# yakir12/PawsomeTracker.jl

Measured on AMD Instinct MI355X. Metric: DoG+argmax frames/s, 1080p 256x256 windows batch 4096; % HBM roofline @1/8 GPU, higher is better.
Workload: dtype f32

## Files before the change

pawsometracker.jl_amd/csrc/dog_prune.hpp:

```cpp
#pragma once
#include "dog_roll.hpp"
#include "dog_prune_words.hpp"
#include "dog_prune_publish.hpp"

namespace pdog {

struct PruneGeo {
    LaunchGeo g;
    double kinv;
    float tmax;
    int darker;
    unsigned long long *stat;
    uint64_t *host;
    PruneJob *jobs;
    const uint32_t *wq;
};

constexpr int PRUNE_NT = 256;
constexpr int PRUNE_B = 8;
constexpr int PRUNE_PHASES = 9;
constexpr int PRUNE_REFINE_MAX_SPAN = 32;
__host__ __device__ inline int prune_refine_pitch(int NS) { return (NS + 3) / 4 * 4; }
struct PruneLds { size_t cell, E, segd, strd, S, R, patch, root, hull2, total; };
__host__ __device__ inline PruneLds prune_lds(int n1, int n2, int L, int nslots, bool refine = false)
// ... 60 lines not shown

    const int ncols = g.nthin ? g.thin_x0 : g.n2;
    const int ws = min(TW, ncols);
    auto slot_cols = [&](int sl, int &c0, int &c1) {
        const bool strip = sl < g.nstrips;
        c0 = strip ? ((ncols >= TW) ? min(sl * TW, ncols - TW) : 0) : g.thin_x0 + (sl - g.nstrips);
        c1 = c0 + (strip ? ws + L - 1 : L);
    };
    auto seg_id = [&](int c) {
        int id = 0;
        for (int sl = 0; sl < g.nslots; ++sl) {
            int c0, c1;
            slot_cols(sl, c0, c1);
            id += (c0 <= c) + (c1 <= c);
        }
        return id;
    };
    auto row_in = [&](int gi) { return gi >= 0 && gi < g.fh; };
    const bool narrow8 = NARROW && g.fw < 8, narrow4 = NARROW && g.fw < 4;
    const unsigned rs = (unsigned)g.row_stride;
    auto frame_at = [&](int gi, int gjc) { return frame + ((unsigned long long)(unsigned)pw_clamp_row(gi, g.fh) * rs + (unsigned)gjc); };
    auto tile_word = [&](int gi, int gj, uint32_t in) -> uint32_t {
        uint32_t w = 0;
        if (in == 0xffffffffu) {
            __builtin_memcpy(&w, frame + (long long)gi * g.row_stride + gj, 4);
        } else if (in) {
#pragma unroll
            for (int i = 0; i < 4; ++i)
                if ((in >> (8 * i)) & 1u) w |= (uint32_t)frame[(long long)gi * g.row_stride + gj + i] << (8 * i);
        }
        return w;
    };

    const int nitems = nsub * ncx;
    auto cell_load = [&](int band, int cx, uint32_t (&w)[2 * CH]) {
        const int gj = wj0 + 8 * cx, gi0 = ti0 + band * CH;
        if (!narrow8) {
            const uint8_t *src = frame_at(gi0, pw_clamp_col(gj, g.fw, 8));
#pragma unroll
            for (int r = 0; r < CH; ++r) {
                __builtin_memcpy(&w[2 * r], src, 8);
                src += (unsigned)(gi0 + r) < (unsigned)(g.fh - 1) ? rs : 0u;
            }
        } else {
            const uint32_t in_a = pw_mask(gj, 0, g.fw), in_b = pw_mask(gj + 4, 0, g.fw);
            for (int r = 0; r < CH; ++r) {
                const bool rin = row_in(gi0 + r);
                w[2 * r] = tile_word(gi0 + r, gj, rin ? in_a : 0u);
                w[2 * r + 1] = tile_word(gi0 + r, gj + 4, rin ? in_b : 0u);
            }
        }
    };

    if (tid == 0) s_nstr = 0;
    int dc;
    uint32_t cur[2 * CH];
    {
        constexpr int DCN = 1024 / NT;
        const int tH = NA, tW = TWin;
        int sv[DCN];
        bool sin[DCN];
#pragma unroll
        for (int j = 0; j < DCN; ++j) {
            const int k = tid + j * NT;
            const int gi = ti0 + (int)(((long long)(k >> 5) * tH) >> 5), gj = wj0 + (int)(((long long)(k & 31) * tW) >> 5);
            sin[j] = row_in(gi) && gj >= 0 && gj < g.fw;
            sv[j] = *frame_at(gi, min(max(gj, 0), g.fw - 1));
        }
        {
            const int it0 = min(tid, nitems - 1), band0 = it0 / ncx;
            cell_load(band0, it0 - band0 * ncx, cur);
        }
        for (int i = tid; i < nsub * nseg * 2; i += NT) S[i] = 0;
        if (refine) {
            for (int i = tid; i <= nsub; i += NT) root[i * rp + ncx] = 0;
            for (int i = tid; i < ncx; i += NT) root[nsub * rp + i] = 0;
        }
        int sum = 0;
#pragma unroll
        for (int j = 0; j < DCN; ++j) sum += sin[j] ? sv[j] : g.fill;
        sum = wave_sum(sum);
        if (lane == 0) s_sum[wave] = sum;
        __syncthreads();
        int tot = 0;
        for (int w = 0; w < NW; ++w) tot += s_sum[w];
        dc = __builtin_amdgcn_readfirstlane(dc_from_sum(tot, g.fill));
    }
    for (int d = tid; d < TQ2; d += NT) {
        int sd = -1;
        if (4 * d < TWin) {
            const int first = seg_id(4 * d), last = seg_id(min(4 * d + 3, TWin - 1));
            if (first == last) sd = first;
            else strd[atomicAdd(&s_nstr, 1)] = (unsigned short)d;
        }
        segd[d] = (short)sd;
    }
    __syncthreads();
    PRUNE_STAMP(0);

    PwAcc ext = pw_init();
    auto cell_sums = [&](int band, int cx, const uint32_t (&w)[2 * CH]) {
        const int col0 = 8 * cx, gj = wj0 + col0, a0 = band * CH, gi0 = ti0 + a0, nr = min(CH, NA - a0);
        const uint32_t cnt_a = pw_mask(col0, 0, TWin), cnt_b = pw_mask(col0 + 4, 0, TWin);
        uint32_t s2a = 0, s1a = 0, s2b = 0, s1b = 0;
        if (nr == CH && gi0 >= 0 && gi0 + CH <= g.fh && gj >= 0 && gj + 8 <= g.fw) {
#pragma unroll
            for (int r = 0; r < CH; ++r) {
                const PwWords xa = pw_words(w[2 * r], 0xffffffffu, cnt_a, fill4), xb = pw_words(w[2 * r + 1], 0xffffffffu, cnt_b, fill4);
                pw_moments(s2a, s1a, xa.wz);
                pw_extremes(ext, xa);
                pw_moments(s2b, s1b, xb.wz);
                pw_extremes(ext, xb);
            }
        } else {
            const uint32_t in_a = pw_mask(gj, 0, g.fw), in_b = pw_mask(gj + 4, 0, g.fw);
            if ((in_a | in_b) == 0u || gi0 >= g.fh || gi0 + nr <= 0) {
                const PwWords xa = pw_words(0u, 0u, cnt_a, fill4), xb = pw_words(0u, 0u, cnt_b, fill4);
                pw_moments(s2a, s1a, xa.wz);
                pw_moments(s2b, s1b, xb.wz);
                s2a *= (uint32_t)nr; s1a *= (uint32_t)nr; s2b *= (uint32_t)nr; s1b *= (uint32_t)nr;
                pw_extremes(ext, xa);
                pw_extremes(ext, xb);
            } else {
                const PwShift sh = narrow8 ? PwShift{0u, 0u} : pw_shift(pw_clamp_col(gj, g.fw, 8) - gj, 8);
#pragma unroll
                for (int r = 0; r < CH; ++r) {
                    const bool rin = row_in(gi0 + r), rc = r < nr;
                    const uint64_t v = pw_rebuild64((uint64_t)w[2 * r] | ((uint64_t)w[2 * r + 1] << 32), sh);
                    const PwWords xa = pw_words((uint32_t)v, rin ? in_a : 0u, rc ? cnt_a : 0u, fill4);
                    const PwWords xb = pw_words((uint32_t)(v >> 32), rin ? in_b : 0u, rc ? cnt_b : 0u, fill4);
                    pw_moments(s2a, s1a, xa.wz);
                    pw_extremes(ext, xa);
                    pw_moments(s2b, s1b, xb.wz);
                    pw_extremes(ext, xb);
                }
            }
        }
        const int npx = nr * min(TWin - col0, 8);
        cell[band * ncx + cx] = pw_sum(s1a + s1b, npx, dc);
        if (refine) root[band * rp + cx] = (unsigned short)pw_root16(pw_energy(s2a + s2b, s1a + s1b, npx, dc));
        const int sda = segd[2 * cx], sdb = segd[2 * cx + 1];
        unsigned *Sb = S + 2 * band * nseg;
        if (sda == sdb) {
            if (sda >= 0) { atomicAdd(Sb + 2 * sda, s2a + s2b); atomicAdd(Sb + 2 * sda + 1, s1a + s1b); }
        } else {
            if (sda >= 0) { atomicAdd(Sb + 2 * sda, s2a); atomicAdd(Sb + 2 * sda + 1, s1a); }
            if (sdb >= 0) { atomicAdd(Sb + 2 * sdb, s2b); atomicAdd(Sb + 2 * sdb + 1, s1b); }
        }
    };
    if (tid < nitems) {
        int band = tid / ncx, cx = tid - band * ncx;
        const int bstep = NT / ncx, cstep = NT - bstep * ncx;
        for (int it = tid + NT; it < nitems; it += NT) {
            int nband = band + bstep, ncell = cx + cstep;
            if (ncell >= ncx) { ncell -= ncx; ++nband; }
            uint32_t nxt[2 * CH];
            cell_load(nband, ncell, nxt);
            cell_sums(band, cx, cur);
#pragma unroll
            for (int i = 0; i < 2 * CH; ++i) cur[i] = nxt[i];
            band = nband;
            cx = ncell;
        }
        cell_sums(band, cx, cur);
    }
    {
        const int pmax = wave_reduce_bits(pw_pmax(ext), [](int a, int c) { return a > c ? a : c; });
        const int pmin = wave_min(pw_pmin(ext));
        if (lane == 0) { s_pmax[wave] = pmax; s_pmin[wave] = pmin; }
    }
    __syncthreads();
    PRUNE_STAMP(1);

    for (int j = 0, nstr = s_nstr; j < nstr; ++j) {
        const int d = strd[j], gj = wj0 + 4 * d;
        const uint32_t in_cols = pw_mask(gj, 0, g.fw);
        const int gjc = narrow4 ? 0 : pw_clamp_col(gj, g.fw, 4);
        const PwShift sh = narrow4 ? PwShift{0u, 0u} : pw_shift(gjc - gj, 4);
        for (int t = tid; t < 4 * nsub; t += NT) {
            const int band = t >> 2, col = 4 * d + (t & 3), a0 = band * CH, nr = min(CH, NA - a0);
            if (col >= TWin) continue;
            const uint32_t counted = pw_mask(4 * d, col, col + 1);
            uint32_t w[CH];
            if (!narrow4) {
#pragma unroll
                for (int r = 0; r < CH; ++r) __builtin_memcpy(&w[r], frame_at(ti0 + a0 + r, gjc), 4);
            } else {
                for (int r = 0; r < CH; ++r) w[r] = tile_word(ti0 + a0 + r, gj, row_in(ti0 + a0 + r) ? in_cols & counted : 0u);
// ... 291 lines not shown
```

pawsometracker.jl_amd/csrc/dog_prune_words.hpp:

```cpp
#pragma once
#include <stdint.h>

#if defined(__HIPCC__) || defined(__CUDACC__)
#define PW_HD __host__ __device__ inline
#else
#define PW_HD inline
#endif

namespace pdog {

PW_HD uint32_t pw_low_bytes(int n) { return n >= 4 ? 0xffffffffu : n <= 0 ? 0u : (1u << (8 * n)) - 1u; }
PW_HD uint32_t pw_mask(int col0, int lo, int hi) { return pw_low_bytes(hi - col0) & ~pw_low_bytes(lo - col0); }

struct PwWords { uint32_t wz, wo; };
PW_HD PwWords pw_words(uint32_t w, uint32_t in_frame, uint32_t counted, uint32_t fill4)
{
    const uint32_t keep = in_frame & counted;
    const uint32_t z = (w & keep) | (fill4 & counted & ~keep);
    return PwWords{z, z | ~counted};
}

PW_HD int pw_clamp_col(int gj, int fw, int width) { return gj < 0 ? 0 : gj > fw - width ? fw - width : gj; }
PW_HD int pw_clamp_row(int gi, int fh) { return gi < 0 ? 0 : gi > fh - 1 ? fh - 1 : gi; }
struct PwShift { unsigned up, down; };
// ... 8 lines not shown
#if defined(__HIP_DEVICE_COMPILE__)
typedef unsigned short pw_us2 __attribute__((ext_vector_type(2)));
PW_HD uint32_t pw_dot4(uint32_t a, uint32_t b, uint32_t c) { return __builtin_amdgcn_udot4(a, b, c, false); }
PW_HD uint32_t pw_pk_max(uint32_t a, uint32_t b)
{
    return __builtin_bit_cast(uint32_t, __builtin_elementwise_max(__builtin_bit_cast(pw_us2, a), __builtin_bit_cast(pw_us2, b)));
}
PW_HD uint32_t pw_pk_min(uint32_t a, uint32_t b)
{
    return __builtin_bit_cast(uint32_t, __builtin_elementwise_min(__builtin_bit_cast(pw_us2, a), __builtin_bit_cast(pw_us2, b)));
}
PW_HD uint32_t pw_mul24(uint32_t a, uint32_t b) { return __umul24(a, b); }
PW_HD float pw_sqrt_est(float x) { return __builtin_amdgcn_sqrtf(x); }
#else
PW_HD uint32_t pw_mul24(uint32_t a, uint32_t b) { return a * b; }
PW_HD float pw_sqrt_est(float x) { return __builtin_sqrtf(x); }
PW_HD uint32_t pw_dot4(uint32_t a, uint32_t b, uint32_t c)
{
    for (int i = 0; i < 4; ++i) c += ((a >> (8 * i)) & 0xffu) * ((b >> (8 * i)) & 0xffu);
    return c;
}
PW_HD uint32_t pw_pk_max(uint32_t a, uint32_t b)
{
    const uint32_t al = a & 0xffffu, bl = b & 0xffffu, ah = a >> 16, bh = b >> 16;
    return (al > bl ? al : bl) | ((ah > bh ? ah : bh) << 16);
}
PW_HD uint32_t pw_pk_min(uint32_t a, uint32_t b)
{
    const uint32_t al = a & 0xffffu, bl = b & 0xffffu, ah = a >> 16, bh = b >> 16;
    return (al < bl ? al : bl) | ((ah < bh ? ah : bh) << 16);
}
#endif

constexpr uint32_t PW_EVEN = 0x00ff00ffu, PW_ODD = 0xff00ff00u;

struct PwAcc {
    uint32_t s2, s1;
    uint32_t max_e, max_o, min_e, min_o;
};
PW_HD PwAcc pw_init() { return PwAcc{0u, 0u, 0u, 0u, PW_EVEN, PW_ODD}; }

PW_HD void pw_moments(uint32_t &s2, uint32_t &s1, uint32_t wz)
{
    s2 = pw_dot4(wz, wz, s2);
    s1 = pw_dot4(wz, 0x01010101u, s1);
}
PW_HD void pw_extremes(PwAcc &a, PwWords x)
{
    a.max_e = pw_pk_max(a.max_e, x.wz & PW_EVEN);
    a.max_o = pw_pk_max(a.max_o, x.wz & PW_ODD);
    a.min_e = pw_pk_min(a.min_e, x.wo & PW_EVEN);
    a.min_o = pw_pk_min(a.min_o, x.wo & PW_ODD);
}
PW_HD void pw_update(PwAcc &a, PwWords x)
{
    pw_moments(a.s2, a.s1, x.wz);
    pw_extremes(a, x);
}

PW_HD int pw_pmax(const PwAcc &a)
{
    const uint32_t e = (a.max_e & 0xffffu) > (a.max_e >> 16) ? (a.max_e & 0xffffu) : (a.max_e >> 16);
    const uint32_t o = (a.max_o & 0xffffu) > (a.max_o >> 16) ? (a.max_o & 0xffffu) : (a.max_o >> 16);
    return (int)(e > (o >> 8) ? e : (o >> 8));
}
PW_HD int pw_pmin(const PwAcc &a)
{
    const uint32_t e = (a.min_e & 0xffffu) < (a.min_e >> 16) ? (a.min_e & 0xffffu) : (a.min_e >> 16);
    const uint32_t o = (a.min_o & 0xffffu) < (a.min_o >> 16) ? (a.min_o & 0xffffu) : (a.min_o >> 16);
    return (int)(e < (o >> 8) ? e : (o >> 8));
}

PW_HD uint32_t pw_energy(uint32_t s2, uint32_t s1, int n, int dc) { return (s2 + (uint32_t)n * (uint32_t)(dc * dc)) - 2u * (uint32_t)dc * s1; }
PW_HD uint32_t pw_root16(uint32_t e)
{
    const uint32_t e256 = e << 8;
    uint32_t r = (uint32_t)(16.0f * pw_sqrt_est((float)e));
    r += pw_mul24(r, r) < e256;
    r += pw_mul24(r, r) < e256;
    return r;
}
PW_HD int pw_sum(uint32_t s1, int n, int dc) { return (int)s1 - n * dc; }
PW_HD int pw_V(int pmax, int pmin, int dc)
{
    const int up = pmax - dc, dn = dc - pmin, v = up > dn ? up : dn;
    return v > 0 ? v : 0;
}

}
```

pawsometracker.jl_amd/csrc/pawsome_dog.hip:

```cpp
#include "pdog_host.hpp"
#include "pdog_mailbox.hpp"
#include "pdog_policy.hpp"
#include "pdog_plan.hpp"
#include "dog_kernels.hpp"
#include "dog_roll.hpp"
#include "dog_prune.hpp"
#include "dog_twopass.hpp"
#include "dog_fused.hpp"
#include "dog_exact.hpp"
#include "dog_tiled.hpp"
#include "dog_measure.hpp"
#include "dog_step.hpp"

#include <algorithm>
#include <cmath>
#include <cstdio>
#include <cstring>
#include <cstdlib>
#include <atomic>
#include <chrono>
#include <map>
#include <memory>
#include <mutex>
#include <thread>
// ... 200 lines not shown
    hipEvent_t ev_h2d[kSlots] = {nullptr, nullptr, nullptr}, ev_used[kSlots] = {nullptr, nullptr, nullptr};
};

}

struct pdog_tracker {
    int device = 0;
    Switches sw;
    hipEvent_t ev_switch = nullptr;
    int fh = 0, fw = 0, r1 = 0, r2 = 0, n1 = 0, n2 = 0, L = 0, fill = 0, darker = 0;
    double tw = 0, sigma = 0;
    Plan plan;
    const VariantKernels *kern = nullptr;
    int fused_resident = 0, tiled_resident = 0;
    DeviceBuffer<int32_t> d_chain_tmp;
    pdog::StagedTable table;
    TiledRun tiled_run;
    DeviceBuffer<f2> d_V;
    MapPolicy map_policy;
    unsigned win_launched = 0;
    PrunePolicy prune_policy;
    double K_norm = 0;
    DeviceBuffer<unsigned long long> d_prune_stat;
    DeviceBuffer<uint32_t> d_refine_wq;
    int last_prune_n = 0, last_prune_nstrips = 0;
    DeviceBuffer<PruneJob> d_prune_jobs;
    int last_n = 0, last_nslots = 0;
    DeviceBuffer<float> d_map;
    DeviceBuffer<int> d_dc;
    DeviceBuffer<int> d_counter;
    hipStream_t own_stream = nullptr, stream = nullptr;
    hipStream_t aux_stream = nullptr;
    hipEvent_t ev_fork = nullptr, ev_join = nullptr;
    DeviceBuffer<f2> d_taps_row, d_taps_col;
    DeviceBuffer<f2> d_taps_roll;
    DeviceBuffer<f2> d_fold_r;
    DeviceBuffer<float> d_part_val, d_part_sec;
    DeviceBuffer<unsigned long long> d_part_mask;
    DeviceBuffer<int> d_part_idx;
    bool exact = true;
    bool exact_all = false;
    std::vector<double> h_gp, h_gm;
    double F_sym_int = 0, F_sym_sep = 0, F_ring = 0, F_rescan = 0;
    DeviceBuffer<double> d_K64;
    DeviceBuffer<double> d_g64;
    DeviceBuffer<RefineParams> d_rp;
    double exact_T64 = 0.0;
    DeviceBuffer<unsigned long long> d_ref_stat;
    DeviceBuffer<uint8_t> d_frame;
    DeviceBuffer<int32_t> d_small;
    PinnedBuffer<Mailbox> h_pinned{hipHostMallocMapped | hipHostMallocCoherent};
    int32_t ticket = 0;
    DeviceBuffer<float> d_resp;
    PinnedBuffer<uint8_t> h_tile{hipHostMallocMapped};
    Ingest ingest;
    pdog::PeaksState peaks;
    pdog::GroupWalkState exclusive;
    pdog::GroupWalkState motion;
    bool motion_lds = false;
    pdog::PredictState predict;

    ~pdog_tracker()
    {
        (void)hipSetDevice(device);
        if (stream) (void)hipStreamSynchronize(stream);
        for (hipStream_t s : {ingest.stream, aux_stream})
            if (s) { (void)hipStreamSynchronize(s); (void)hipStreamDestroy(s); }
        for (int k = 0; k < Ingest::kSlots; ++k)
            for (hipEvent_t e : {ingest.ev_h2d[k], ingest.ev_used[k]})
                if (e) (void)hipEventDestroy(e);
        for (hipEvent_t e : {ev_fork, ev_join, ev_switch})
            if (e) (void)hipEventDestroy(e);
        if (own_stream) (void)hipStreamDestroy(own_stream);
    }
};

pdog::PeaksState *pdog::peaks_state(pdog_tracker *t)
{
    t->peaks.device = t->device;
    t->peaks.map_cap = t->sw.map_cap;
    return &t->peaks;
}

pdog::GroupWalkState *pdog::exclusive_state(pdog_tracker *t)
{
    t->exclusive.device = t->device;
    return &t->exclusive;
}

pdog::GroupWalkState *pdog::motion_state(pdog_tracker *t)
{
    t->motion.device = t->device;
    return &t->motion;
}

bool pdog::motion_lds(const pdog_tracker *t) { return t->motion_lds; }

pdog::PredictState *pdog::predict_state(pdog_tracker *t)
{
    t->predict.device = t->device;
    return &t->predict;
}

namespace {
// ... 459 lines not shown
        fin.done_flag = req.done_flag;
        fin.done_value = req.done_value;
        return launch_finish(t, g, fin);
    }
    if (t->exact && !t->exact_all && hr == 8 && t->L >= TWOPASS_FLUSH_L) tg.vmax = t->d_dc.get() + t->d_dc.capacity() / 2;
    hipLaunchKernelGGL(dog_dc_kernel, dim3(n), dim3(64), 0, t->stream, g, t->d_dc.get(), tg.vmax);
    HIP_TRY(hipGetLastError());
    const tp_fn h1 = h1_kernel(t, false);
    const tp_fn hp = hr == 8 ? hpass8_kernel(t, want_resp, false) : want_resp ? (tp_fn)dog_hpass_kernel<13, 16, true> : (tp_fn)dog_hpass_kernel<13, 16, false>;
    for (int w0 = 0; w0 < n; w0 += chunk) {
        const int nw = std::min(chunk, n - w0);
        tg.win0 = w0;
        hipLaunchKernelGGL(h1, dim3(nw * tg.h1blocks_per_win), dim3(256), l1, t->stream, tg, tr);
        HIP_TRY(hipGetLastError());
        hipLaunchKernelGGL(hp, dim3(nw * tg.hblocks_per_win), dim3(256), l2, t->stream, tg, tc);
        HIP_TRY(hipGetLastError());
    }
    fin.vmax = tg.vmax;
    return launch_finish(t, g, fin);
}

#ifndef PDOG_PRUNE_XCD_GROUP
#define PDOG_PRUNE_XCD_GROUP 1
#endif
constexpr int kPruneXcdGroup = PDOG_PRUNE_XCD_GROUP;
static_assert(kPruneXcdGroup >= 1 && (kPruneXcdGroup & (kPruneXcdGroup - 1)) == 0, "a power of two");
constexpr size_t kPruneMaxLds = 64 * 1024;
bool use_pruning(pdog_tracker *t, bool want_resp, int nslots)
{
    if (!t->kern->fn_prune || want_resp || t->exact_all || t->sw.no_prune || prune_lds(t->n1, t->n2, t->L, nslots).total > kPruneMaxLds) return false;
    return t->prune_policy.decide(__atomic_load_n(&t->h_pinned.get()->prune_pub, __ATOMIC_ACQUIRE));
}

int launch_strips(pdog_tracker *t, const Request &req, LaunchGeo g)
{
    const VariantShape &v = *t->plan.shape;
    const VariantKernels &k = *t->kern;
    const Plan &plan = t->plan;
    const bool roll = v.family == Family::Roll;
    const int n = req.n;
    int grid = round_up(g.nblocks, 8);
    if (t->exact && !t->exact_all) {
        const KernelWords &kw = t->h_pinned.get()->kernel;
        const uint32_t flagged = __atomic_load_n(&kw.flagged, __ATOMIC_ACQUIRE);
        t->map_policy.observe(flagged, __atomic_load_n(&kw.finished, __ATOMIC_ACQUIRE));
        if (!g.resp && t->map_policy.on() && !t->sw.no_roll_map)
            if (int rc = reserve_response_map(t, g)) return rc;
    }
    const bool want_resp = g.resp != nullptr;
    const int NA = t->n1 + t->L - 1;
    const size_t fold_wave_lds = (size_t)(NA + FOLD_GO) * sizeof(f2);
    const bool prune = use_pruning(t, want_resp, g.nslots);
    const bool fold = roll && roll_folds(v.LT) && plan.nthin == 1 && !want_resp && !prune && !t->sw.no_fold && (plan.nstrips >= 8 || t->sw.fold_always) &&
                      (size_t)FINISH_WPB * fold_wave_lds <= kMaxLds - 1024;
    const f2 *tr = t->d_taps_row.get(), *tc = t->d_taps_col.get();
    if (prune) {
        PruneGeo pg;
        pg.g = g;
        const int nsub = (t->n1 + t->L - 1 + ROLL_CH - 1) / ROLL_CH;
        pg.g.prune = (t->sw.fenced_publish || !pp_fits(n, g.nstrips, g.nslots, nsub)) ? PRUNE_FENCED_PUBLISH : 0;
        pg.kinv = 255.0 / t->K_norm;
        pg.tmax = std::max(g.ex.T, g.ex.T_rescan);
        pg.darker = t->darker;
        pg.stat = t->d_prune_stat.get();
        pg.host = &t->h_pinned.device()->prune_pub;
        if (int rc = t->d_prune_jobs.reserve((size_t)g.nblocks + 1, &t->stream)) return rc;
        pg.jobs = t->d_prune_jobs.get();
        const bool refine = !t->sw.no_refine && prune_span(t->L) <= PRUNE_REFINE_MAX_SPAN && prune_lds(t->n1, t->n2, t->L, g.nslots, true).total <= kPruneMaxLds;
        pg.wq = refine ? t->d_refine_wq.get() : nullptr;
        hipLaunchKernelGGL(t->fw < 8 ? dog_prune_kernel<true> : dog_prune_kernel<false>, dim3(n), dim3(PRUNE_NT), prune_lds(t->n1, t->n2, t->L, g.nslots, refine).total, t->stream, pg, tr, tc);
        t->last_prune_n = n;
        t->last_prune_nstrips = g.nstrips;
        HIP_TRY(hipGetLastError());
        static_assert((kPruneXcdGroup & ~PRUNE_GROUP_MASK) == 0, "the group size shares its word with PRUNE_NO_RANGE_END");
        g.prune = kPruneXcdGroup | (t->sw.no_range_end ? PRUNE_NO_RANGE_END : 0);
        grid = round_up(g.nblocks, 8 * kPruneXcdGroup);
    }
    if (fold) {
        if (int rc = t->d_fold_r.reserve((size_t)n * NA, &t->stream)) return rc;
        g.fold_r = t->d_fold_r.get();
    } else if (plan.nthin) {
        HIP_TRY(hipEventRecord(t->ev_fork, t->stream));
        HIP_TRY(hipStreamWaitEvent(t->aux_stream, t->ev_fork, 0));
        const size_t thin_lds = thin_lds_bytes(t->n1, t->L);
        hipLaunchKernelGGL(want_resp ? k.thin_resp : k.thin, dim3(round_up(n * plan.nthin, 8)), dim3(256), thin_lds, t->aux_stream, g, tr, tc);
        HIP_TRY(hipGetLastError());
        HIP_TRY(hipEventRecord(t->ev_join, t->aux_stream));
    }
    size_t lds_bytes = v.lds(t->L);
#ifdef PDOG_ABLATIONS
    if (t->sw.lds_pad) {
        lds_bytes += (size_t)t->sw.lds_pad;
        (void)raise_lds_limit((const void *)(want_resp ? k.fn_resp : k.fn), lds_bytes);
    }
#endif
    kernel_fn fn = want_resp ? k.fn_resp : prune ? k.fn_prune : k.fn;
    if (!want_resp && !prune && roll && v.LT == 65 && v.id == 100) {
        const int cls = roll_epi_class(t->n1, 65);
#define PDOG_EPI_PICK(C) if (cls == C) fn = (kernel_fn)dog_roll_kernel<65, false, 0, C>;
        PDOG_EPI_CLASSES(PDOG_EPI_PICK)
#undef PDOG_EPI_PICK
    }
    {
        LaunchGeo gs = g;
        if (prune) gs.jobs = t->d_prune_jobs.get();
        hipLaunchKernelGGL(fn, dim3(grid), dim3(v.NT), lds_bytes, t->stream, gs, tr, roll ? (const f2 *)t->d_taps_roll.get() : tc);
    }
    HIP_TRY(hipGetLastError());
    if (plan.nthin && !fold) HIP_TRY(hipStreamWaitEvent(t->stream, t->ev_join, 0));
    const int covered = plan.nthin ? plan.thin_x0 : t->n2;
    t->last_n = n;
    t->last_nslots = g.nslots;
    Finish fin;
    fin.slot_w = v.tw();
    if (roll) fin.slot_last = std::max(0, covered - v.tw());
    fin.use_mask = roll;
    fin.map = g.resp;
    fin.out_ij = req.out_ij;
    return launch_finish(t, g, fin);
}

int launch_detect(pdog_tracker *t, const Request &req, bool *ticket_armed = nullptr)
{
    const VariantShape &v = *t->plan.shape;
    const Plan &plan = t->plan;
    if (ticket_armed) *ticket_armed = false;
    const int path = path_for_batch(plan, t->sw, req.n);
    if (path == kPathFused || path == kPathTiled) {
        Request one = req;
        if (req.n != 1) one.dc_host = -1;
        bool launched = true;
        if (path == kPathFused) {
            if (int rc = launch_fused(t, one)) return rc;
        } else if (int rc = launch_tiled(t, one, &launched)) return rc;
        if (launched) {
            if (ticket_armed) *ticket_armed = req.done_flag != nullptr;
            return PDOG_OK;
        }
    }
    LaunchGeo g = base_geo(t, req);
    use_partials(t, g);
    g.ex = exact_ctl(t, (v.family == Family::Roll ? kFamRoll : kFamRing));
// ... 274 lines not shown
    if (!t) return fail(PDOG_E_ARG, "pdog_sync: null tracker");
    return drain_and_check(t, "pdog_sync");
}

int pdog_set_exact(pdog_tracker *t, int on)
{
    if (!t) return fail(PDOG_E_ARG, "pdog_set_exact: null tracker");
    if (on && !exact_fits(geometry_of(t)))
        return fail(PDOG_E_ARG, "pdog_set_exact: window too tall for the refinement's LDS block");
    HIP_TRY(hipStreamSynchronize(t->stream));
    t->exact = on != 0;
    t->exact_all = on == 2;
    return PDOG_OK;
}

int pdog_set_tuning(pdog_tracker *t, const char *key, int value)
{
    if (!t || !key) return fail(PDOG_E_ARG, "pdog_set_tuning: null pointer");
    HIP_TRY(hipSetDevice(t->device));
    HIP_TRY(hipStreamSynchronize(t->stream));
    const std::string k(key);
    const bool on = value != 0;
    if (k == "host_copy") t->sw.host_copy = on;
    else if (k == "host_sync") t->sw.host_sync = on;
    else if (k == "twopass_4l") t->sw.twopass_4l = on;
    else if (k == "no_roll_map") t->sw.no_roll_map = on;
    else if (k == "no_fold") t->sw.no_fold = on;
    else if (k == "fold_always") t->sw.fold_always = on;
    else if (k == "no_pad_skip") t->sw.no_pad_skip = on;
    else if (k == "no_prune") t->sw.no_prune = on;
    else if (k == "no_refine") t->sw.no_refine = on;
    else if (k == "no_range_end") t->sw.no_range_end = on;
    else if (k == "fenced_publish") t->sw.fenced_publish = on;
    else if (k == "fault_inject") t->sw.fault_inject = on;
    else if (k == "measure_global") t->sw.measure_global = on;
    else if (k == "peaks_no_list") t->peaks.no_list = on;
    else if (k == "motion_lds") t->motion_lds = on;
    else if (k == "no_fused_c" || k == "no_tiled") {
        Switches sw = t->sw;
        (k == "no_tiled" ? sw.no_tiled : sw.no_fused_c) = on;
        return replan(t, sw, t->plan.forced ? t->plan.shape->id : -1);
    } else return fail(PDOG_E_ARG, "pdog_set_tuning: unknown key '" + k + "'");
    return PDOG_OK;
}

int pdog_get_exact_detail(pdog_tracker *t, uint64_t out[4])
{
    if (!t || !out) return fail(PDOG_E_ARG, "pdog_get_exact_detail: null pointer");
    if (int rc = drain_and_check(t, "pdog_get_exact_detail")) return rc;
    unsigned long long v[16];
    HIP_TRY(hipMemcpy(v, t->d_ref_stat.get(), sizeof v, hipMemcpyDeviceToHost));
    for (int i = 0; i < 4; ++i) out[i] = (uint64_t)v[i];
#ifdef PDOG_ABLATIONS
    std::fprintf(stderr, "pdog refine phases (shader cycles, thread 0): setup %llu, tile %llu, row32 %llu, col32 %llu, row64 %llu, cand64 %llu, verdict %llu\n",
                 v[8], v[9], v[10], v[11], v[12], v[13], v[14]);
#endif
    return PDOG_OK;
}

int pdog_get_prune_counts(pdog_tracker *t, uint64_t out[2])
{
    if (!t || !out) return fail(PDOG_E_ARG, "pdog_get_prune_counts: null pointer");
    if (int rc = drain_and_check(t, "pdog_get_prune_counts")) return rc;
    unsigned long long v[2];
    HIP_TRY(hipMemcpy(v, t->d_prune_stat.get(), sizeof v, hipMemcpyDeviceToHost));
    out[0] = (uint64_t)v[0];
    out[1] = (uint64_t)v[1];
#ifdef PDOG_ABLATIONS
    {
        unsigned long long ph[PRUNE_PHASES + 1];
        HIP_TRY(hipMemcpy(ph, t->d_prune_stat.get() + 4, sizeof ph, hipMemcpyDeviceToHost));
        const double wg = ph[PRUNE_PHASES] ? (double)ph[PRUNE_PHASES] : 1.0;
        std::fprintf(stderr, "pdog prune phases (cycles per workgroup, thread 0; %llu workgroups): dc %.0f, energy %.0f, straddle %.0f, cell+E %.0f, patch %.0f, row %.0f, "
                             "col %.0f, hull %.0f, publish %.0f\n",
                     ph[PRUNE_PHASES], ph[0] / wg, ph[1] / wg, ph[2] / wg, ph[3] / wg, ph[4] / wg, ph[5] / wg, ph[6] / wg, ph[7] / wg, ph[8] / wg);
    }
#endif
    return PDOG_OK;
}

int pdog_get_prune_jobs(pdog_tracker *t, int capacity, int32_t *h_out, int *count)
{
    if (!t || !count || capacity < 0 || (capacity > 0 && !h_out)) return fail(PDOG_E_ARG, "pdog_get_prune_jobs: bad argument");
    if (int rc = drain_and_check(t, "pdog_get_prune_jobs")) return rc;
    if (t->last_prune_n <= 0) return fail(PDOG_E_ARG, "pdog_get_prune_jobs: no batch of this tracker ran the bounding pass");
    PruneJob head;
    HIP_TRY(hipMemcpy(&head, t->d_prune_jobs.get(), sizeof head, hipMemcpyDeviceToHost));
    const long long room = (long long)t->last_prune_n * t->last_prune_nstrips;
    if (head.b < 0 || head.b > room) return fail(PDOG_E_RANGE, "pdog_get_prune_jobs: the list's count lies outside the list");
    *count = head.b;
    const int m = std::min(head.b, capacity);
    std::vector<PruneJob> jobs((size_t)m);
    if (m) HIP_TRY(hipMemcpy(jobs.data(), t->d_prune_jobs.get() + 1, sizeof(PruneJob) * (size_t)m, hipMemcpyDeviceToHost));
    for (int i = 0; i < m; ++i) {
        h_out[4 * i] = jobs[i].b;
        h_out[4 * i + 1] = jobs[i].s_dc & 0xffff;
        h_out[4 * i + 2] = jobs[i].ba;
        h_out[4 * i + 3] = jobs[i].bb;
    }
    return PDOG_OK;
}

int pdog_get_batch_maxima(pdog_tracker *t, int n, float *h_out)
{
    if (!t || !h_out || n <= 0) return fail(PDOG_E_ARG, "pdog_get_batch_maxima: bad argument");
    if (int rc = drain_and_check(t, "pdog_get_batch_maxima")) return rc;
    if (n != t->last_n || t->last_nslots <= 0) return fail(PDOG_E_ARG, "pdog_get_batch_maxima: the last batch on the strip kernels had another size (or there was none)");
    std::vector<float> pv((size_t)n * t->last_nslots);
    HIP_TRY(hipMemcpy(pv.data(), t->d_part_val.get(), sizeof(float) * pv.size(), hipMemcpyDeviceToHost));
    for (int b = 0; b < n; ++b) h_out[b] = *std::max_element(pv.begin() + (size_t)b * t->last_nslots, pv.begin() + (size_t)(b + 1) * t->last_nslots);
    return PDOG_OK;
}

int pdog_get_exact(pdog_tracker *t, int *out_on, double *out_threshold, uint64_t *out_refined)
{
    if (!t) return fail(PDOG_E_ARG, "pdog_get_exact: null tracker");
    if (out_on) *out_on = t->exact ? 1 : 0;
    if (out_threshold) {
        *out_threshold = (double)exact_ctl(t, batch_family(*t->plan.shape)).T;
    }
    if (out_refined) {
        if (int rc = drain_and_check(t, "pdog_get_exact")) return rc;
        unsigned long long v = 0;
        HIP_TRY(hipMemcpy(&v, t->d_ref_stat.get(), sizeof v, hipMemcpyDeviceToHost));
        *out_refined = (uint64_t)v;
    }
    return PDOG_OK;
}

int pdog_detect_batch(pdog_tracker *t, const uint8_t *d_frames, int64_t frame_stride, int64_t row_stride,
                      int n_frames, const int32_t *d_frame_index, const int32_t *d_guesses, int n,
                      int32_t *d_out_ij, float *d_out_resp)
// ... 495 lines not shown
```

pawsometracker.jl_amd/csrc/pdog_plan.hpp:

```cpp
#pragma once
#include "../../include/pawsome_dog.h"
#include "dog_layout.hpp"
#include "dog_roll_range.hpp"

#include <algorithm>
#include <cmath>
#include <cstddef>
#include <initializer_list>
#include <string>
#include <vector>

namespace pdog {

struct Switches {
    size_t scratch_cap = (size_t)6 << 30;
    size_t map_cap = (size_t)4 << 30;
    int host_threads = 0;
    int ingest_chunk = 0;
    bool host_copy = false;
    bool host_sync = false;
    bool twopass_4l = false;
    bool no_tiled = false;
    bool no_roll_map = false;
    bool no_fold = false;
    bool fold_always = false;
    bool no_pad_skip = false;
    bool no_prune = false;
    bool no_refine = false;
    bool no_range_end = false;
    bool fenced_publish = false;
    bool no_fused_c = false;
    bool measure_global = false;
    bool fault_inject = false;
    bool host_trace = false, hpass16 = false, ingest_no_nt = false, ingest_trace = false, fused_diag = false;
    bool tiled_force = false;
    bool no_host_dc = false;
    int tiled_sub = 0;
    int tp_ph1 = 0, tp_php = 0;
    int v_after = 64;
    int h1_u = 4;
    int hp_u = 8;
    int tiled_batch = 2;
    int fused_pr = 0, fused_pc = 0;
    int lds_pad = 0;
};

struct Geometry {
    int fh = 0, fw = 0, n1 = 0, n2 = 0, L = 0;
};

constexpr int kPathFused = 300, kPathTwoPass = 200, kPathTiled = 400;
constexpr size_t kMaxLds = 160 * 1024;
constexpr int kThinMax = 6;
enum class Family { Ring, Roll, TwoPass, Fused };
struct VariantShape {
    int id;
    Family family;
    int P, XG, Q, CH, LT, NT;
    bool full_set;
    constexpr int tw() const { return P * XG; }
    constexpr int ring(int L) const { return LT ? ring_rows(CH, LT, Q) : ring_rows(CH, L, Q); }
    constexpr int pa(int L) const { return pitch_a(tw() + L - 1); }
    constexpr size_t lds(int L) const
// ... 256 lines not shown
        return PDOG_OK;
    }
    if (best->full_set && g.n2 > best->tw()) {
        const int r = g.n2 % best->tw();
        const size_t thin_lds = thin_lds_bytes(g.n1, g.L);
        if (r > 0 && r <= kThinMax && thin_lds <= kMaxLds - 1024) {
            p.lds.thin = thin_lds;
            p.nthin = r;
            p.thin_x0 = g.n2 - r;
            p.nstrips = p.thin_x0 / best->tw();
        }
    }
    p.lds.batch = best->lds(g.L);
    *out = p;
    return PDOG_OK;
}

inline bool exact_fits(const Geometry &g) { return refine_lds_bytes(g.n1, g.L, 1, 8) <= kMaxLds - 8192; }

inline int path_for_batch(const Plan &p, const Switches &sw, int n)
{
    const VariantShape &v = *p.shape;
    const bool twopass = v.family == Family::TwoPass;
    if (v.family == Family::Fused) return kPathFused;
    if (p.forced) return twopass ? kPathTwoPass : v.id;
    const bool few = twopass ? n <= 256 : ((long long)n * (p.nstrips + (p.nthin ? 1 : 0)) < 1200 || (long long)p.geo.n1 * p.geo.n2 < 3000);
    if (sw.tiled_force && p.tiled.ok && n <= sw.tiled_batch) return kPathTiled;
    if (few && p.fused.ok) return kPathFused;
    if (p.tiled.ok && n <= sw.tiled_batch) return kPathTiled;
    if (twopass || (few && p.small_twopass)) return kPathTwoPass;
    return v.id;
}

inline bool tiled_serves(const Plan &p, int resident, int n, int chain_len)
{
    return p.tiled.ok && n >= 1 && (chain_len <= 1 || (long long)n * p.tiled.ns1 * p.tiled.ns2 <= resident);
}

inline int chain_strips(const Geometry &g) { return (g.n2 + ROLL_TW - 1) / ROLL_TW; }

enum class ChainPath { Fused, Persistent, Tiled, Stepped };

inline ChainPath chain_path(const Plan &p, const Switches &, int tiled_resident, int n_clips, int n_steps, bool table, bool progress)
{
    const VariantShape &v = *p.shape;
    if (table && n_steps == 1) return ChainPath::Stepped;
    const long long strip_waves = (long long)n_clips * chain_strips(p.geo);
    const bool fused_wins = p.fused.ok && !p.forced && ((long long)p.geo.n1 * p.geo.n2 < 3000 || strip_waves < 1400);
    const bool persistent = !progress && v.full_set && chain_strips(p.geo) <= 8 && !fused_wins &&
                            (p.forced || !p.small_twopass || strip_waves >= 1000);
    if (v.family == Family::Fused || (!persistent && !p.forced && p.fused.ok)) return ChainPath::Fused;
    if (persistent) return ChainPath::Persistent;
    if (!p.forced && tiled_serves(p, tiled_resident, n_clips, n_steps)) return ChainPath::Tiled;
    return ChainPath::Stepped;
}

enum KernelFamily : int { kFamRoll, kFamRing, kFamFused, kFamTwoPass8, kFamTwoPass16 };
inline KernelFamily batch_family(const VariantShape &v)
{
    return v.family == Family::Roll ? kFamRoll : v.family == Family::TwoPass ? kFamTwoPass8 : v.family == Family::Fused ? kFamFused : kFamRing;
}
inline double twopass_factor(const Plan &p, const Switches &sw, bool hr8, double F_sym_sep, const std::vector<double> &gp, const std::vector<double> &gm)
{
    if (!hr8 || p.geo.L < TWOPASS_FLUSH_L) return F_sym_sep;
    const int l = p.geo.L, H = l / 2;
    const int U1 = sw.h1_u, m_r = twopass_ring(p.tp_ph1, U1), U2 = hr8 ? sw.hp_u : 16, m_c = hr8 ? twopass_ring(p.tp_php, U2) : twopass_ring(13, 16);
// ... 40 lines not shown
```

Measured before the change: 14.66 million.

## Add chunked prune pipeline and a fast path for whole interior cells

The bounding prepass now iterates whole 8-column cells first and handles the ragged last column separately. Fully interior whole cells skip the pw_words masking and update the packed extremes directly with shifts instead of even/odd masks, which trims ALU work in the hot loop. Separately, a chunked launch path lets the prune kernel of one chunk overlap the next chunk's prepass on an auxiliary stream, with the thin-strip kernel on its own stream. With kPruneChunkMax = 1 the default chunk count stays 1, so the chunking is only reachable through the new prune_chunk tuning switch.

```diff
diff --git a/pawsometracker.jl_amd/csrc/dog_prune.hpp b/pawsometracker.jl_amd/csrc/dog_prune.hpp
--- a/pawsometracker.jl_amd/csrc/dog_prune.hpp
+++ b/pawsometracker.jl_amd/csrc/dog_prune.hpp
@@ -116,7 +116,11 @@
         return w;
     };
 
-    const int nitems = nsub * ncx;
+    const int ncxf = TWin / 8, nitems = nsub * ncx, nwhole = nsub * ncxf;
+    auto item_cell = [&](int it, int &band, int &cx) {
+        if (it < nwhole) { band = it / ncxf; cx = it - band * ncxf; }
+        else { band = it - nwhole; cx = ncxf; }
+    };
     auto cell_load = [&](int band, int cx, uint32_t (&w)[2 * CH]) {
         const int gj = wj0 + 8 * cx, gi0 = ti0 + band * CH;
         if (!narrow8) {
@@ -152,8 +156,9 @@
             sv[j] = *frame_at(gi, min(max(gj, 0), g.fw - 1));
         }
         {
-            const int it0 = min(tid, nitems - 1), band0 = it0 / ncx;
-            cell_load(band0, it0 - band0 * ncx, cur);
+            int band0, cx0;
+            item_cell(min(tid, nitems - 1), band0, cx0);
+            cell_load(band0, cx0, cur);
         }
         for (int i = tid; i < nsub * nseg * 2; i += NT) S[i] = 0;
         if (refine) {
@@ -187,7 +192,16 @@
         const int col0 = 8 * cx, gj = wj0 + col0, a0 = band * CH, gi0 = ti0 + a0, nr = min(CH, NA - a0);
         const uint32_t cnt_a = pw_mask(col0, 0, TWin), cnt_b = pw_mask(col0 + 4, 0, TWin);
         uint32_t s2a = 0, s1a = 0, s2b = 0, s1b = 0;
-        if (nr == CH && gi0 >= 0 && gi0 + CH <= g.fh && gj >= 0 && gj + 8 <= g.fw) {
+        const bool inside = nr == CH && gi0 >= 0 && gi0 + CH <= g.fh && gj >= 0 && gj + 8 <= g.fw;
+        if (inside && cx < ncxf) {
+#pragma unroll
+            for (int r = 0; r < CH; ++r) {
+                pw_moments(s2a, s1a, w[2 * r]);
+                pw_extremes(ext, w[2 * r]);
+                pw_moments(s2b, s1b, w[2 * r + 1]);
+                pw_extremes(ext, w[2 * r + 1]);
+            }
+        } else if (inside) {
 #pragma unroll
             for (int r = 0; r < CH; ++r) {
                 const PwWords xa = pw_words(w[2 * r], 0xffffffffu, cnt_a, fill4), xb = pw_words(w[2 * r + 1], 0xffffffffu, cnt_b, fill4);
@@ -233,11 +247,13 @@
         }
     };
     if (tid < nitems) {
-        int band = tid / ncx, cx = tid - band * ncx;
-        const int bstep = NT / ncx, cstep = NT - bstep * ncx;
+        int band, cx;
+        item_cell(tid, band, cx);
+        const int bstep = NT / ncxf, cstep = NT - bstep * ncxf;
         for (int it = tid + NT; it < nitems; it += NT) {
             int nband = band + bstep, ncell = cx + cstep;
-            if (ncell >= ncx) { ncell -= ncx; ++nband; }
+            if (ncell >= ncxf) { ncell -= ncxf; ++nband; }
+            if (it >= nwhole) { nband = it - nwhole; ncell = ncxf; }
             uint32_t nxt[2 * CH];
             cell_load(nband, ncell, nxt);
             cell_sums(band, cx, cur);
diff --git a/pawsometracker.jl_amd/csrc/dog_prune_words.hpp b/pawsometracker.jl_amd/csrc/dog_prune_words.hpp
--- a/pawsometracker.jl_amd/csrc/dog_prune_words.hpp
+++ b/pawsometracker.jl_amd/csrc/dog_prune_words.hpp
@@ -64,25 +64,31 @@
 }
 #endif
 
-constexpr uint32_t PW_EVEN = 0x00ff00ffu, PW_ODD = 0xff00ff00u;
-
 struct PwAcc {
     uint32_t s2, s1;
-    uint32_t max_e, max_o, min_e, min_o;
+    uint32_t max_o, max_e, min_o, min_e;
 };
-PW_HD PwAcc pw_init() { return PwAcc{0u, 0u, 0u, 0u, PW_EVEN, PW_ODD}; }
+PW_HD PwAcc pw_init() { return PwAcc{0u, 0u, 0u, 0u, 0xffffffffu, 0xffffffffu}; }
 
 PW_HD void pw_moments(uint32_t &s2, uint32_t &s1, uint32_t wz)
 {
     s2 = pw_dot4(wz, wz, s2);
     s1 = pw_dot4(wz, 0x01010101u, s1);
 }
+PW_HD void pw_extremes(PwAcc &a, uint32_t w)
+{
+    const uint32_t e = w << 8;
+    a.max_o = pw_pk_max(a.max_o, w);
+    a.max_e = pw_pk_max(a.max_e, e);
+    a.min_o = pw_pk_min(a.min_o, w);
+    a.min_e = pw_pk_min(a.min_e, e);
+}
 PW_HD void pw_extremes(PwAcc &a, PwWords x)
 {
-    a.max_e = pw_pk_max(a.max_e, x.wz & PW_EVEN);
-    a.max_o = pw_pk_max(a.max_o, x.wz & PW_ODD);
-    a.min_e = pw_pk_min(a.min_e, x.wo & PW_EVEN);
-    a.min_o = pw_pk_min(a.min_o, x.wo & PW_ODD);
+    a.max_o = pw_pk_max(a.max_o, x.wz);
+    a.max_e = pw_pk_max(a.max_e, x.wz << 8);
+    a.min_o = pw_pk_min(a.min_o, x.wo);
+    a.min_e = pw_pk_min(a.min_e, x.wo << 8);
 }
 PW_HD void pw_update(PwAcc &a, PwWords x)
 {
@@ -92,15 +98,13 @@
 
 PW_HD int pw_pmax(const PwAcc &a)
 {
-    const uint32_t e = (a.max_e & 0xffffu) > (a.max_e >> 16) ? (a.max_e & 0xffffu) : (a.max_e >> 16);
-    const uint32_t o = (a.max_o & 0xffffu) > (a.max_o >> 16) ? (a.max_o & 0xffffu) : (a.max_o >> 16);
-    return (int)(e > (o >> 8) ? e : (o >> 8));
+    const uint32_t o = pw_pk_max(a.max_o, a.max_o << 16), e = pw_pk_max(a.max_e, a.max_e << 16);
+    return (int)((o > e ? o : e) >> 24);
 }
 PW_HD int pw_pmin(const PwAcc &a)
 {
-    const uint32_t e = (a.min_e & 0xffffu) < (a.min_e >> 16) ? (a.min_e & 0xffffu) : (a.min_e >> 16);
-    const uint32_t o = (a.min_o & 0xffffu) < (a.min_o >> 16) ? (a.min_o & 0xffffu) : (a.min_o >> 16);
-    return (int)(e < (o >> 8) ? e : (o >> 8));
+    const uint32_t o = pw_pk_min(a.min_o, a.min_o << 16), e = pw_pk_min(a.min_e, a.min_e << 16);
+    return (int)((o < e ? o : e) >> 24);
 }
 
 PW_HD uint32_t pw_energy(uint32_t s2, uint32_t s1, int n, int dc) { return (s2 + (uint32_t)n * (uint32_t)(dc * dc)) - 2u * (uint32_t)dc * s1; }
diff --git a/pawsometracker.jl_amd/csrc/pawsome_dog.hip b/pawsometracker.jl_amd/csrc/pawsome_dog.hip
--- a/pawsometracker.jl_amd/csrc/pawsome_dog.hip
+++ b/pawsometracker.jl_amd/csrc/pawsome_dog.hip
@@ -256,6 +256,9 @@
     hipStream_t own_stream = nullptr, stream = nullptr;
     hipStream_t aux_stream = nullptr;
     hipEvent_t ev_fork = nullptr, ev_join = nullptr;
+    hipStream_t thin_stream = nullptr;
+    hipEvent_t ev_join_thin = nullptr;
+    PruneChunks last_prune_chunks;
     DeviceBuffer<f2> d_taps_row, d_taps_col;
     DeviceBuffer<f2> d_taps_roll;
     DeviceBuffer<f2> d_fold_r;
@@ -288,12 +291,12 @@
     {
         (void)hipSetDevice(device);
         if (stream) (void)hipStreamSynchronize(stream);
-        for (hipStream_t s : {ingest.stream, aux_stream})
+        for (hipStream_t s : {ingest.stream, aux_stream, thin_stream})
             if (s) { (void)hipStreamSynchronize(s); (void)hipStreamDestroy(s); }
         for (int k = 0; k < Ingest::kSlots; ++k)
             for (hipEvent_t e : {ingest.ev_h2d[k], ingest.ev_used[k]})
                 if (e) (void)hipEventDestroy(e);
-        for (hipEvent_t e : {ev_fork, ev_join, ev_switch})
+        for (hipEvent_t e : {ev_fork, ev_join, ev_join_thin, ev_switch})
             if (e) (void)hipEventDestroy(e);
         if (own_stream) (void)hipStreamDestroy(own_stream);
     }
@@ -819,6 +822,70 @@
     return t->prune_policy.decide(__atomic_load_n(&t->h_pinned.get()->prune_pub, __ATOMIC_ACQUIRE));
 }
 
+int launch_prepass(pdog_tracker *t, PruneGeo pg, bool refine, hipStream_t stream)
+{
+    const LaunchGeo &g = pg.g;
+    const int nsub = (t->n1 + t->L - 1 + ROLL_CH - 1) / ROLL_CH;
+    pg.g.prune = (t->sw.fenced_publish || !pp_fits(g.n, g.nstrips, g.nslots, nsub)) ? PRUNE_FENCED_PUBLISH : 0;
+    hipLaunchKernelGGL(t->fw < 8 ? dog_prune_kernel<true> : dog_prune_kernel<false>, dim3(g.n), dim3(PRUNE_NT), prune_lds(t->n1, t->n2, t->L, g.nslots, refine).total, stream, pg,
+                       (const f2 *)t->d_taps_row.get(), (const f2 *)t->d_taps_col.get());
+    HIP_TRY(hipGetLastError());
+    return PDOG_OK;
+}
+
+int launch_prune_chunks(pdog_tracker *t, const PruneGeo &pg, const LaunchGeo &g, const PruneChunks &cuts, bool refine)
+{
+    const VariantShape &v = *t->plan.shape;
+    const VariantKernels &k = *t->kern;
+    if (!t->thin_stream) {
+        HIP_TRY(hipStreamCreateWithFlags(&t->thin_stream, hipStreamNonBlocking));
+        HIP_TRY(hipEventCreateWithFlags(&t->ev_join_thin, hipEventDisableTiming));
+    }
+    auto chunk_of = [](LaunchGeo c, int w0, int nc) {
+        c.guesses += 2 * (size_t)w0;
+        if (c.frame_index) c.frame_index += w0;
+        else c.frames += (long long)w0 * c.frame_stride;
+        const size_t o = (size_t)w0 * c.nslots;
+        c.part_val += o; c.part_idx += o; c.part_sec += o; c.part_mask += o;
+        c.n = nc;
+        c.nblocks = nc * c.nstrips;
+        return c;
+    };
+    const f2 *tr = t->d_taps_row.get(), *tc = t->d_taps_col.get();
+    bool forked = false;
+    auto queue = [&]() -> int {
+        for (int c = 0; c < cuts.count; ++c) {
+            const int w0 = cuts.begin(c), nc = cuts.end(c) - w0;
+            PruneGeo pc = pg;
+            pc.g = chunk_of(pg.g, w0, nc);
+            pc.jobs = pg.jobs + ((size_t)w0 * g.nstrips + c);
+            if (int rc = launch_prepass(t, pc, refine, t->stream)) return rc;
+            HIP_TRY(hipEventRecord(t->ev_fork, t->stream));
+            forked = true;
+            HIP_TRY(hipStreamWaitEvent(t->aux_stream, t->ev_fork, 0));
+            LaunchGeo gs = chunk_of(g, w0, nc);
+            gs.jobs = pc.jobs;
+            hipLaunchKernelGGL(k.fn_prune, dim3(round_up(gs.nblocks, 8 * kPruneXcdGroup)), dim3(v.NT), v.lds(t->L), t->aux_stream, gs, tr, (const f2 *)t->d_taps_roll.get());
+            HIP_TRY(hipGetLastError());
+            if (g.nthin && c == cuts.count - 1) {
+                HIP_TRY(hipStreamWaitEvent(t->thin_stream, t->ev_fork, 0));
+                hipLaunchKernelGGL(k.thin, dim3(round_up(g.n * g.nthin, 8)), dim3(256), thin_lds_bytes(t->n1, t->L), t->thin_stream, g, tr, tc);
+                HIP_TRY(hipGetLastError());
+            }
+        }
+        return PDOG_OK;
+    };
+    const int rc = queue();
+    if (forked) {
+        hipError_t join = hipSuccess;
+        for (hipError_t e : {hipEventRecord(t->ev_join, t->aux_stream), hipStreamWaitEvent(t->stream, t->ev_join, 0), hipEventRecord(t->ev_join_thin, t->thin_stream),
+                             hipStreamWaitEvent(t->stream, t->ev_join_thin, 0)})
+            if (join == hipSuccess) join = e;
+        if (!rc) HIP_TRY(join);
+    }
+    return rc;
+}
+
 int launch_strips(pdog_tracker *t, const Request &req, LaunchGeo g)
 {
     const VariantShape &v = *t->plan.shape;
@@ -841,60 +908,63 @@
     const bool fold = roll && roll_folds(v.LT) && plan.nthin == 1 && !want_resp && !prune && !t->sw.no_fold && (plan.nstrips >= 8 || t->sw.fold_always) &&
                       (size_t)FINISH_WPB * fold_wave_lds <= kMaxLds - 1024;
     const f2 *tr = t->d_taps_row.get(), *tc = t->d_taps_col.get();
+    const PruneChunks cuts = prune_chunks(prune ? n : 0, t->sw.prune_chunk, t->sw.no_prune_overlap);
     if (prune) {
         PruneGeo pg;
         pg.g = g;
-        const int nsub = (t->n1 + t->L - 1 + ROLL_CH - 1) / ROLL_CH;
-        pg.g.prune = (t->sw.fenced_publish || !pp_fits(n, g.nstrips, g.nslots, nsub)) ? PRUNE_FENCED_PUBLISH : 0;
         pg.kinv = 255.0 / t->K_norm;
         pg.tmax = std::max(g.ex.T, g.ex.T_rescan);
         pg.darker = t->darker;
         pg.stat = t->d_prune_stat.get();
         pg.host = &t->h_pinned.device()->prune_pub;
-        if (int rc = t->d_prune_jobs.reserve((size_t)g.nblocks + 1, &t->stream)) return rc;
+        if (int rc = t->d_prune_jobs.reserve((size_t)g.nblocks + cuts.count, &t->stream)) return rc;
         pg.jobs = t->d_prune_jobs.get();
         const bool refine = !t->sw.no_refine && prune_span(t->L) <= PRUNE_REFINE_MAX_SPAN && prune_lds(t->n1, t->n2, t->L, g.nslots, true).total <= kPruneMaxLds;
         pg.wq = refine ? t->d_refine_wq.get() : nullptr;
-        hipLaunchKernelGGL(t->fw < 8 ? dog_prune_kernel<true> : dog_prune_kernel<false>, dim3(n), dim3(PRUNE_NT), prune_lds(t->n1, t->n2, t->L, g.nslots, refine).total, t->stream, pg, tr, tc);
         t->last_prune_n = n;
         t->last_prune_nstrips = g.nstrips;
-        HIP_TRY(hipGetLastError());
+        t->last_prune_chunks = cuts;
         static_assert((kPruneXcdGroup & ~PRUNE_GROUP_MASK) == 0, "the group size shares its word with PRUNE_NO_RANGE_END");
         g.prune = kPruneXcdGroup | (t->sw.no_range_end ? PRUNE_NO_RANGE_END : 0);
-        grid = round_up(g.nblocks, 8 * kPruneXcdGroup);
-    }
-    if (fold) {
-        if (int rc = t->d_fold_r.reserve((size_t)n * NA, &t->stream)) return rc;
-        g.fold_r = t->d_fold_r.get();
-    } else if (plan.nthin) {
-        HIP_TRY(hipEventRecord(t->ev_fork, t->stream));
-        HIP_TRY(hipStreamWaitEvent(t->aux_stream, t->ev_fork, 0));
-        const size_t thin_lds = thin_lds_bytes(t->n1, t->L);
-        hipLaunchKernelGGL(want_resp ? k.thin_resp : k.thin, dim3(round_up(n * plan.nthin, 8)), dim3(256), thin_lds, t->aux_stream, g, tr, tc);
+        if (cuts.count == 1) {
+            if (int rc = launch_prepass(t, pg, refine, t->stream)) return rc;
+            grid = round_up(g.nblocks, 8 * kPruneXcdGroup);
+        } else if (int rc = launch_prune_chunks(t, pg, g, cuts, refine)) return rc;
+    }
+    if (cuts.count == 1) {
+        if (fold) {
+            if (int rc = t->d_fold_r.reserve((size_t)n * NA, &t->stream)) return rc;
+            g.fold_r = t->d_fold_r.get();
+        } else if (plan.nthin) {
+            HIP_TRY(hipEventRecord(t->ev_fork, t->stream));
+            HIP_TRY(hipStreamWaitEvent(t->aux_stream, t->ev_fork, 0));
+            const size_t thin_lds = thin_lds_bytes(t->n1, t->L);
+            hipLaunchKernelGGL(want_resp ? k.thin_resp : k.thin, dim3(round_up(n * plan.nthin, 8)), dim3(256), thin_lds, t->aux_stream, g, tr, tc);
+            HIP_TRY(hipGetLastError());
+            HIP_TRY(hipEventRecord(t->ev_join, t->aux_stream));
+        }
+        size_t lds_bytes = v.lds(t->L);
+#ifdef PDOG_ABLATIONS
+        if (t->sw.lds_pad) {
+            lds_bytes += (size_t)t->sw.lds_pad;
+            (void)raise_lds_limit((const void *)(want_resp ? k.fn_resp : k.fn), lds_bytes);
+        }
+#endif
+        kernel_fn fn = want_resp ? k.fn_resp : prune ? k.fn_prune : k.fn;
+        if (!want_resp && !prune && roll && v.LT == 65 && v.id == 100) {
+            const int cls = roll_epi_class(t->n1, 65);
+#define PDOG_EPI_PICK(C) if (cls == C) fn = (kernel_fn)dog_roll_kernel<65, false, 0, C>;
+            PDOG_EPI_CLASSES(PDOG_EPI_PICK)
+#undef PDOG_EPI_PICK
+        }
+        {
+            LaunchGeo gs = g;
+            if (prune) gs.jobs = t->d_prune_jobs.get();
+            hipLaunchKernelGGL(fn, dim3(grid), dim3(v.NT), lds_bytes, t->stream, gs, tr, roll ? (const f2 *)t->d_taps_roll.get() : tc);
+        }
         HIP_TRY(hipGetLastError());
-        HIP_TRY(hipEventRecord(t->ev_join, t->aux_stream));
-    }
-    size_t lds_bytes = v.lds(t->L);
-#ifdef PDOG_ABLATIONS
-    if (t->sw.lds_pad) {
-        lds_bytes += (size_t)t->sw.lds_pad;
-        (void)raise_lds_limit((const void *)(want_resp ? k.fn_resp : k.fn), lds_bytes);
-    }
-#endif
-    kernel_fn fn = want_resp ? k.fn_resp : prune ? k.fn_prune : k.fn;
-    if (!want_resp && !prune && roll && v.LT == 65 && v.id == 100) {
-        const int cls = roll_epi_class(t->n1, 65);
-#define PDOG_EPI_PICK(C) if (cls == C) fn = (kernel_fn)dog_roll_kernel<65, false, 0, C>;
-        PDOG_EPI_CLASSES(PDOG_EPI_PICK)
-#undef PDOG_EPI_PICK
-    }
-    {
-        LaunchGeo gs = g;
-        if (prune) gs.jobs = t->d_prune_jobs.get();
-        hipLaunchKernelGGL(fn, dim3(grid), dim3(v.NT), lds_bytes, t->stream, gs, tr, roll ? (const f2 *)t->d_taps_roll.get() : tc);
-    }
-    HIP_TRY(hipGetLastError());
-    if (plan.nthin && !fold) HIP_TRY(hipStreamWaitEvent(t->stream, t->ev_join, 0));
+        if (plan.nthin && !fold) HIP_TRY(hipStreamWaitEvent(t->stream, t->ev_join, 0));
+    }
     const int covered = plan.nthin ? plan.thin_x0 : t->n2;
     t->last_n = n;
     t->last_nslots = g.nslots;
@@ -1235,6 +1305,11 @@
     else if (k == "no_refine") t->sw.no_refine = on;
     else if (k == "no_range_end") t->sw.no_range_end = on;
     else if (k == "fenced_publish") t->sw.fenced_publish = on;
+    else if (k == "no_prune_overlap") t->sw.no_prune_overlap = on;
+    else if (k == "prune_chunk") {
+        if (value < 0) return fail(PDOG_E_ARG, "pdog_set_tuning: prune_chunk is a number of windows, or 0 for the rule");
+        t->sw.prune_chunk = value;
+    }
     else if (k == "fault_inject") t->sw.fault_inject = on;
     else if (k == "measure_global") t->sw.measure_global = on;
     else if (k == "peaks_no_list") t->peaks.no_list = on;
@@ -1287,20 +1362,25 @@
     if (!t || !count || capacity < 0 || (capacity > 0 && !h_out)) return fail(PDOG_E_ARG, "pdog_get_prune_jobs: bad argument");
     if (int rc = drain_and_check(t, "pdog_get_prune_jobs")) return rc;
     if (t->last_prune_n <= 0) return fail(PDOG_E_ARG, "pdog_get_prune_jobs: no batch of this tracker ran the bounding pass");
-    PruneJob head;
-    HIP_TRY(hipMemcpy(&head, t->d_prune_jobs.get(), sizeof head, hipMemcpyDeviceToHost));
-    const long long room = (long long)t->last_prune_n * t->last_prune_nstrips;
-    if (head.b < 0 || head.b > room) return fail(PDOG_E_RANGE, "pdog_get_prune_jobs: the list's count lies outside the list");
-    *count = head.b;
-    const int m = std::min(head.b, capacity);
-    std::vector<PruneJob> jobs((size_t)m);
-    if (m) HIP_TRY(hipMemcpy(jobs.data(), t->d_prune_jobs.get() + 1, sizeof(PruneJob) * (size_t)m, hipMemcpyDeviceToHost));
-    for (int i = 0; i < m; ++i) {
-        h_out[4 * i] = jobs[i].b;
-        h_out[4 * i + 1] = jobs[i].s_dc & 0xffff;
-        h_out[4 * i + 2] = jobs[i].ba;
-        h_out[4 * i + 3] = jobs[i].bb;
-    }
+    const PruneChunks &cuts = t->last_prune_chunks;
+    const int ns = t->last_prune_nstrips;
+    std::vector<PruneJob> lists((size_t)t->last_prune_n * ns + cuts.count);
+    HIP_TRY(hipMemcpy(lists.data(), t->d_prune_jobs.get(), sizeof(PruneJob) * lists.size(), hipMemcpyDeviceToHost));
+    int total = 0;
+    for (int c = 0; c < cuts.count; ++c) {
+        const int w0 = cuts.begin(c);
+        const PruneJob *list = lists.data() + ((size_t)w0 * ns + c);
+        const long long room = (long long)(cuts.end(c) - w0) * ns;
+        if (list[0].b < 0 || list[0].b > room) return fail(PDOG_E_RANGE, "pdog_get_prune_jobs: the list's count lies outside the list");
+        for (int i = 1; i <= list[0].b; ++i, ++total) {
+            if (total >= capacity) continue;
+            h_out[4 * total] = w0 + list[i].b;
+            h_out[4 * total + 1] = list[i].s_dc & 0xffff;
+            h_out[4 * total + 2] = list[i].ba;
+            h_out[4 * total + 3] = list[i].bb;
+        }
+    }
+    *count = total;
     return PDOG_OK;
 }
 
diff --git a/pawsometracker.jl_amd/csrc/pdog_plan.hpp b/pawsometracker.jl_amd/csrc/pdog_plan.hpp
--- a/pawsometracker.jl_amd/csrc/pdog_plan.hpp
+++ b/pawsometracker.jl_amd/csrc/pdog_plan.hpp
@@ -29,6 +29,8 @@
     bool no_refine = false;
     bool no_range_end = false;
     bool fenced_publish = false;
+    bool no_prune_overlap = false;
+    int prune_chunk = 0;
     bool no_fused_c = false;
     bool measure_global = false;
     bool fault_inject = false;
@@ -351,6 +353,26 @@
     return v.id;
 }
 
+constexpr int kPruneChunkMin = 1024;
+constexpr int kPruneChunkMax = 1;
+struct PruneChunks {
+    int n = 0, count = 1;
+    int size = 0;
+    int begin(int c) const { return size ? (int)std::min<long long>(n, (long long)c * size) : (int)((long long)n * c / count); }
+    int end(int c) const { return begin(c + 1); }
+};
+inline PruneChunks prune_chunks(int n, int forced, bool single)
+{
+    PruneChunks p;
+    p.n = n;
+    if (single || n <= 0) return p;
+    if (forced > 0) {
+        p.count = (int)(((long long)n + forced - 1) / forced);
+        p.size = forced;
+    } else p.count = std::max(1, std::min(kPruneChunkMax, n / kPruneChunkMin));
+    return p;
+}
+
 inline bool tiled_serves(const Plan &p, int resident, int n, int chain_len)
 {
     return p.tiled.ok && n >= 1 && (chain_len <= 1 || (long long)n * p.tiled.ns1 * p.tiled.ns2 <= resident);
```

Result: no change. 14.79 million (median of 6 runs) (+0.9%).
